# isarandi/smplfitter

Hardware: AMD Instinct MI355X
Metric: fits/sec (SMPL 6890-vert, 3 iters) (higher is better)
Workload: dtype f32; 1 GPU; SMPL-neutral (synthetic SMPL-shaped model) batch 4096/GPU, 6890 verts, num_iter=3, beta_reg=1, joints given; batch_per_gpu=4096, num_iter=3, parallelism=batch-sharded x1

## Files before the change

smplfitter_amd/csrc/kernels_wave.inc:

```
template <bool WEIGHTED>
__global__ __launch_bounds__(256) void k_center_sort_partsum(DevModel m, const float* __restrict__ tv,
                                                             const float* __restrict__ tj,
                                                             const float* __restrict__ vw,
                                                             Workspace ws) {
  extern __shared__ __attribute__((aligned(16))) float smem[];
  const int b = blockIdx.x, tid = threadIdx.x, lane = tid & 63, wave = tid >> 6;
  const int V = m.V, J = m.J, Vp = m.Vp;
  float(*red)[4] = reinterpret_cast<float(*)[4]>(smem + 4 * J * sf::kPsum);
  float* mu = smem + 4 * J * sf::kPsum + 16;
  const float* tvb = tv + (size_t)b * V * 3;
  float sx = 0.f, sy = 0.f, sz = 0.f;
  for (int v = tid; v < V; v += 256) {
    sx += tvb[v * 3];
    sy += tvb[v * 3 + 1];
    sz += tvb[v * 3 + 2];
  }
  if (tj) {
    for (int j = tid; j < J; j += 256) {
      sx += tj[((size_t)b * J + j) * 3];
      sy += tj[((size_t)b * J + j) * 3 + 1];
      sz += tj[((size_t)b * J + j) * 3 + 2];
    }
  }
  sx = wave_sum(sx);
// ... 333 lines not shown
      } else {
        acc[0][0] = __builtin_amdgcn_mfma_f32_32x32x2f32(a0, b0, acc[0][0], 0, 0, 0);
        acc[0][1] = __builtin_amdgcn_mfma_f32_32x32x2f32(a0, b1, acc[0][1], 0, 0, 0);
        acc[1][0] = __builtin_amdgcn_mfma_f32_32x32x2f32(a1, b0, acc[1][0], 0, 0, 0);
        acc[1][1] = __builtin_amdgcn_mfma_f32_32x32x2f32(a1, b1, acc[1][1], 0, 0, 0);
      }
    };
    __builtin_amdgcn_sched_group_barrier(0x100, 8, 0);
    mfma4(a0l.x, a1l.x, b0l.x, b1l.x);
    mfma4(a0l.y, a1l.y, b0l.y, b1l.y);
    mfma4(a0l.z, a1l.z, b0l.z, b1l.z);
    mfma4(a0l.w, a1l.w, b0l.w, b1l.w);
    mfma4(a0h.x, a1h.x, b0h.x, b1h.x);
    mfma4(a0h.y, a1h.y, b0h.y, b1h.y);
    mfma4(a0h.z, a1h.z, b0h.z, b1h.z);
    mfma4(a0h.w, a1h.w, b0h.w, b1h.w);
    if (it + 1 < nk) sstore(buf ^ 1);
    __syncthreads();
  }
#pragma unroll
  for (int mi = 0; mi < 2; ++mi)
#pragma unroll
    for (int ni = 0; ni < 2; ++ni)
#pragma unroll
      for (int r = 0; r < 16; ++r) {
        if (TRANSPOSED) {
          const int inst = m0 + wm + mi * 32 + l31;
          const int n = n0 + wn + ni * 32 + (r & 3) + 8 * (r >> 2) + 4 * lk;
          st_stream<2>(C + ((size_t)(inst >> 6) * N + n) * 64 + (inst & 63), acc[mi][ni][r]);
        } else {
          const int row = m0 + wm + mi * 32 + (r & 3) + 8 * (r >> 2) + 4 * lk;
          const int col = n0 + wn + ni * 32 + l31;
          st_stream<2>(C + (size_t)row * N + col, acc[mi][ni][r]);
        }
      }
}

constexpr int kNW = 4;

template <int NK2, bool TRANSPOSED>
__global__ __launch_bounds__(256, 2) void k_posedirs_gemm_as(const float* __restrict__ A,
                                                          const float* __restrict__ Bsw,
                                                          float* __restrict__ C, int N,
                                                          int tiles_per_chunk, int Mp) {
  constexpr int KP = 2 * NK2, RS = KP + 4;
  constexpr int TILE_F4 = 32 * KP / 4;
  constexpr int NQ = NK2 / 4;
  static_assert(NQ % 2 == 0, "the fragment reads alternate between two register quads");
  extern __shared__ __attribute__((aligned(16))) float smem[];
  const int tid = threadIdx.x, lane = tid & 63, wave = tid >> 6;
  const int l31 = lane & 31, lk = lane >> 5;
  const int m0 = (blockIdx.y * 4 + wave) * 32;
  const int ntiles = N / 32;
  const int t_begin = blockIdx.x * tiles_per_chunk;
  const int t_end = min(t_begin + tiles_per_chunk, ntiles);
  float a[NK2];
  {
    const float4* src = reinterpret_cast<const float4*>(A + (size_t)(m0 + l31) * KP + lk * NK2);
#pragma unroll
    for (int q = 0; q < NK2 / 4; ++q) {
      const float4 v = src[q];
      a[4 * q] = v.x; a[4 * q + 1] = v.y; a[4 * q + 2] = v.z; a[4 * q + 3] = v.w;
    }
  }
  static_assert(TILE_F4 <= 7 * 256, "tile too large for the staging registers");
  float4 s0, s1, s2, s3, s4, s5, s6;
#define SF_STAGE_ALL(OP) OP(0, s0) OP(1, s1) OP(2, s2) OP(3, s3) OP(4, s4) OP(5, s5) OP(6, s6)
  auto gload = [&](int tile) {
    const float4* src = reinterpret_cast<const float4*>(Bsw) + (size_t)tile * TILE_F4;
#define SF_LD(q, r)                                                       \
  if constexpr (256 * (q + 1) <= TILE_F4) r = src[tid + 256 * q];         \
  else if (tid + 256 * q < TILE_F4) r = src[tid + 256 * q];
    SF_STAGE_ALL(SF_LD)
#undef SF_LD
  };
  auto sstore = [&](int buf) {
    float* base = smem + (size_t)buf * 32 * RS;
#define SF_ST(q, r)                                                                        \
  if (256 * (q + 1) <= TILE_F4 || tid + 256 * q < TILE_F4) {                               \
    const int f = tid + 256 * q;                                                           \
    *reinterpret_cast<float4*>(base + (f / (KP / 4)) * RS + 4 * (f % (KP / 4))) = r;      \
  }
    SF_STAGE_ALL(SF_ST)
#undef SF_ST
  };
#undef SF_STAGE_ALL
  if (t_begin >= t_end) return;
  gload(t_begin);
  sstore(0);
  __syncthreads();
  for (int t = t_begin; t < t_end; ++t) {
    const int buf = (t - t_begin) & 1;
    if (t + 1 < t_end) gload(t + 1);
    f32x16 acc;
#pragma unroll
    for (int r = 0; r < 16; ++r) acc[r] = 0.f;
    const float4* brow = reinterpret_cast<const float4*>(smem + (size_t)buf * 32 * RS + l31 * RS + lk * NK2);
    auto mfma4 = [&](const float4& bq, int q) {
      if (TRANSPOSED) {
        acc = __builtin_amdgcn_mfma_f32_32x32x2f32(bq.x, a[4 * q], acc, 0, 0, 0);
        acc = __builtin_amdgcn_mfma_f32_32x32x2f32(bq.y, a[4 * q + 1], acc, 0, 0, 0);
        acc = __builtin_amdgcn_mfma_f32_32x32x2f32(bq.z, a[4 * q + 2], acc, 0, 0, 0);
        acc = __builtin_amdgcn_mfma_f32_32x32x2f32(bq.w, a[4 * q + 3], acc, 0, 0, 0);
      } else {
        acc = __builtin_amdgcn_mfma_f32_32x32x2f32(a[4 * q], bq.x, acc, 0, 0, 0);
        acc = __builtin_amdgcn_mfma_f32_32x32x2f32(a[4 * q + 1], bq.y, acc, 0, 0, 0);
        acc = __builtin_amdgcn_mfma_f32_32x32x2f32(a[4 * q + 2], bq.z, acc, 0, 0, 0);
        acc = __builtin_amdgcn_mfma_f32_32x32x2f32(a[4 * q + 3], bq.w, acc, 0, 0, 0);
      }
    };
    float4 bA = brow[0], bB;
    __builtin_amdgcn_sched_group_barrier(0x100, 1, 0);
#pragma unroll
    for (int q = 0; q < NQ; q += 2) {
      bB = brow[q + 1];
      __builtin_amdgcn_sched_group_barrier(0x100, 1, 0);
      mfma4(bA, q);
      __builtin_amdgcn_sched_group_barrier(0x008, 4, 0);
      if (q + 2 < NQ) bA = brow[q + 2];
      __builtin_amdgcn_sched_group_barrier(0x100, 1, 0);
      mfma4(bB, q + 1);
      __builtin_amdgcn_sched_group_barrier(0x008, 4, 0);
    }
    if (TRANSPOSED) {
      float* ccol = C + ((size_t)(m0 >> 6) * N + t * 32) * 64 + (m0 & 63) + l31;
#pragma unroll
      for (int r = 0; r < 16; ++r)
        st_stream<2>(ccol + (size_t)((r & 3) + 8 * (r >> 2) + 4 * lk) * 64, acc[r]);
    } else {
      float* crow = C + (size_t)m0 * N + t * 32 + l31;
#pragma unroll
      for (int r = 0; r < 16; ++r)
        st_stream<2>(crow + (size_t)((r & 3) + 8 * (r >> 2) + 4 * lk) * N, acc[r]);
    }
    if (t + 1 < t_end) sstore(buf ^ 1);
    __syncthreads();
  }
}

typedef __bf16 bf16x8 __attribute__((ext_vector_type(8)));
constexpr int kGemmKS = 13;
constexpr int kGemmPlaneBytes = 32 * 208 * 2;
constexpr int kGemmTileBytes = sf::kGemm3 ? 2 * kGemmPlaneBytes + 32 * 32 : 3 * kGemmPlaneBytes;
#ifndef SMPLFIT_GEMM_WAVES
#define SMPLFIT_GEMM_WAVES 8
#endif
constexpr int kGemmWaves = SMPLFIT_GEMM_WAVES;
#ifndef SMPLFIT_GEMM_RING
#define SMPLFIT_GEMM_RING 2
#endif
constexpr int kGemmRing = SMPLFIT_GEMM_RING;
static_assert(kGemmRing >= 2 && 16 * (kGemmRing - 1) + (kGemmRing - 2) * (kGemmTileBytes / 1024 / kGemmWaves + 1) <= 63,
              "s_waitcnt vmcnt is a 6-bit count");
template <int N>
__device__ __forceinline__ void wait_vmcnt() {
  asm volatile("s_waitcnt vmcnt(%0)" ::"n"(N) : "memory");
}
constexpr bool kGemm3 = sf::kGemm3;

__device__ __forceinline__ void lds_dma16(const char* src, uint32_t lane_off, char* lds) {
  const uint32_t l = (uint32_t)(uintptr_t)(__attribute__((address_space(3))) char*)lds;
  asm volatile("s_mov_b32 m0, %0\n\ts_nop 0\n\tglobal_load_lds_dwordx4 %1, %2" ::"s"(l), "v"(lane_off), "s"(src) : "memory", "m0");
}

template <bool TRANSPOSED>
__global__ __launch_bounds__(64 * kGemmWaves, 2) void k_posedirs_gemm_bf16x3(const float* __restrict__ A,
                                                                           const uint16_t* __restrict__ Bimg,
                                                                           float* __restrict__ C, int N,
                                                                           int tiles_per_chunk, int Mp) {
  constexpr int KS = kGemmKS, KP = 16 * KS, NW = kGemmWaves;
  constexpr int NDMA = kGemmTileBytes / 1024;
  extern __shared__ __attribute__((aligned(16))) char smem_b[];
  asm volatile("v_mov_b32 v255, 0" ::: "v255");
  const int tid = threadIdx.x, lane = tid & 63;
  const int wave = __builtin_amdgcn_readfirstlane(tid >> 6);
  const int l31 = lane & 31, kg = lane >> 5;
  const int m0 = (blockIdx.y * NW + wave) * 32;
  const bool active = m0 < Mp;
  const int ntiles = N / 32;
  const int t_begin = blockIdx.x * tiles_per_chunk;
  const int t_end = min(t_begin + tiles_per_chunk, ntiles);
  if (t_begin >= t_end) return;
  auto dma_tile = [&](int tile, int buf) {
    const char* src = reinterpret_cast<const char*>(Bimg) + (size_t)tile * kGemmTileBytes;
    char* dst = smem_b + buf * kGemmTileBytes;
#pragma unroll
    for (int i = 0; i < NDMA / NW; ++i) {
      const int c = wave + NW * i;
      lds_dma16(src + c * 1024, lane * 16, dst + c * 1024);
    }
    if (wave < NDMA % NW) {
      const int c = wave + NW * (NDMA / NW);
      lds_dma16(src + c * 1024, lane * 16, dst + c * 1024);
    }
  };
  constexpr int LEAD = kGemmRing - 1;
#pragma unroll
  for (int q = 0; q < LEAD; ++q) dma_tile(min(t_begin + q, t_end - 1), q);
  bf16x8 f1[KS], f2[KS], f3[KS];
  {
    const float* src = A + (size_t)((active ? m0 : 0) + l31) * KP + kg * 8;
#pragma unroll
    for (int s = 0; s < KS; ++s) {
      const float4 lo = *reinterpret_cast<const float4*>(src + 16 * s);
      const float4 hi = *reinterpret_cast<const float4*>(src + 16 * s + 4);
      const float x[8] = {lo.x, lo.y, lo.z, lo.w, hi.x, hi.y, hi.z, hi.w};
#pragma unroll
      for (int j = 0; j < 8; ++j) {
        const __bf16 h = (__bf16)x[j];
        const float r1 = x[j] - (float)h;
        const __bf16 m = (__bf16)r1;
        const __bf16 l = (__bf16)(r1 - (float)m);
        f1[s][j] = h;
        f2[s][j] = m;
        f3[s][j] = l;
      }
    }
  }
  const int frag_off = l31 * (KP * 2) + ((kg ^ ((l31 >> 3) & 1)) * 16);
  asm volatile("s_waitcnt vmcnt(0)" ::: "memory");
  __builtin_amdgcn_s_barrier();
  const bool extra = wave < NDMA % NW;
  int buf = 0, buf_req = LEAD;
  for (int t = t_begin; t < t_end; ++t) {
    const bool more = t + 1 < t_end;
    dma_tile(min(t + LEAD, t_end - 1), buf_req);
    if (active) {
      f32x16 acc;
#pragma unroll
      for (int r = 0; r < 16; ++r) acc[r] = 0.f;
      const char* base = smem_b + buf * kGemmTileBytes + frag_off;
      auto frag = [&](int plane, int s) {
        if constexpr (kGemm3) {
          if (plane == 2) return *reinterpret_cast<const bf16x8*>(smem_b + buf * kGemmTileBytes + 2 * kGemmPlaneBytes + l31 * 32 + kg * 16);
        }
        return *reinterpret_cast<const bf16x8*>(base + plane * kGemmPlaneBytes + s * 32);
      };
      auto mm = [&](const bf16x8& p, const bf16x8& f) {
        if (TRANSPOSED) acc = __builtin_amdgcn_mfma_f32_32x32x16_bf16(p, f, acc, 0, 0, 0);
        else acc = __builtin_amdgcn_mfma_f32_32x32x16_bf16(f, p, acc, 0, 0, 0);
      };
      bf16x8 p1 = frag(0, 0), p2 = frag(1, 0), p3 = p1;
      if constexpr (!kGemm3) p3 = frag(2, 0);
#pragma unroll
      for (int s = 0; s < KS; ++s) {
        bf16x8 n1, n2, n3;
        if (s + 1 < KS) {
          n1 = frag(0, s + 1);
          n2 = frag(1, s + 1);
          n3 = n1;
          if (!kGemm3 || s + 1 == KS - 1) n3 = frag(2, s + 1);
        }
        if constexpr (kGemm3) {
          if (s == KS - 1) mm(p3, f1[s]);
          mm(p2, f1[s]);
          mm(p1, f2[s]);
          mm(p1, f1[s]);
        } else {
          mm(p3, f1[s]);
          mm(p2, f2[s]);
          mm(p1, f3[s]);
          mm(p2, f1[s]);
          mm(p1, f2[s]);
          mm(p1, f1[s]);
        }
        if (s + 1 < KS) {
          p1 = n1;
          p2 = n2;
          p3 = n3;
        }
      }
      if (TRANSPOSED) {
        float* ccol = C + ((size_t)(m0 >> 6) * N + t * 32) * 64 + (m0 & 63) + l31;
#pragma unroll
        for (int r = 0; r < 16; ++r) st_stream<2>(ccol + (size_t)((r & 3) + 8 * (r >> 2) + 4 * kg) * 64, acc[r]);
      } else {
        float* crow = C + (size_t)m0 * N + t * 32 + l31;
#pragma unroll
        for (int r = 0; r < 16; ++r)
          st_stream<2>(crow + (size_t)((r & 3) + 8 * (r >> 2) + 4 * kg) * N, acc[r]);
      }
    }
    constexpr int N0 = (LEAD - 1) * (NDMA / NW), N1 = (LEAD - 1) * (NDMA / NW + 1), ST = 16 * LEAD;
    if (!more) wait_vmcnt<0>();
    else if (active) {
      if (extra) wait_vmcnt<ST + N1>();
      else wait_vmcnt<ST + N0>();
    } else {
      if (extra) wait_vmcnt<N1>();
      else wait_vmcnt<N0>();
    }
    __builtin_amdgcn_s_barrier();
    buf_req = buf;
    buf = buf + 1 == kGemmRing ? 0 : buf + 1;
  }
}

constexpr int kTgPlanesA = sf::kGemm3 ? 2 : 3;
constexpr int kTgStageA = kTgPlanesA * 256 * 64;
constexpr int kTgStageB = 3 * 128 * 64;
constexpr int kTgStage = kTgStageA + kTgStageB;

__global__ __launch_bounds__(256) void k_split_features(const float* __restrict__ A, uint16_t* __restrict__ img, int Mrows,
                                                        int Kp, int kc32) {
  const int mt = blockIdx.x, kc = blockIdx.y, r = threadIdx.x, row = mt * 256 + r;
  float x[32];
#pragma unroll
  for (int q = 0; q < 8; ++q) {
    const int k = kc * 32 + 4 * q;
    float4 v = make_float4(0.f, 0.f, 0.f, 0.f);
    if (row < Mrows && k + 3 < Kp) v = *reinterpret_cast<const float4*>(A + (size_t)row * Kp + k);
    else if (row < Mrows) {
      v.x = k < Kp ? A[(size_t)row * Kp + k] : 0.f;
      v.y = k + 1 < Kp ? A[(size_t)row * Kp + k + 1] : 0.f;
      v.z = k + 2 < Kp ? A[(size_t)row * Kp + k + 2] : 0.f;
    }
    x[4 * q] = v.x; x[4 * q + 1] = v.y; x[4 * q + 2] = v.z; x[4 * q + 3] = v.w;
  }
  uint16_t* base = img + ((size_t)mt * kc32 + kc) * (kTgStageA / 2);
#pragma unroll
  for (int sl = 0; sl < 4; ++sl) {
    bf16x8 h, m, l;
#pragma unroll
    for (int j = 0; j < 8; ++j) {
      const float v = x[sl * 8 + j];
      const __bf16 hh = (__bf16)v;
      const float r1 = v - (float)hh;
      const __bf16 mm = (__bf16)r1;
      h[j] = hh; m[j] = mm; l[j] = (__bf16)(r1 - (float)mm);
    }
    const int ps = sl ^ ((r >> 2) & 3);
    uint16_t* d = base + (size_t)r * 32 + ps * 8;
    *reinterpret_cast<bf16x8*>(d) = h;
    *reinterpret_cast<bf16x8*>(d + 256 * 32) = m;
    if constexpr (kTgPlanesA == 3) *reinterpret_cast<bf16x8*>(d + 2 * 256 * 32) = l;
  }
}

constexpr int kTg2B = 2 * 128 * 64;
constexpr int kTg2Bias = kTgStageA + 2 * kTg2B;
constexpr int kTg2Stage = kTg2Bias + 2 * 128 * 64;

__global__ __launch_bounds__(512, 1) void k_posedirs_gemm_bf16x3_tiled(const uint16_t* __restrict__ Aimg,
                                                                       const uint16_t* __restrict__ Bimg,
                                                                       float* __restrict__ C, int N, int Mp, int mt_count,
                                                                       int kc32, int bias_step) {
  static_assert(kGemm3 && kTgPlanesA == 2, "three-product form");
  extern __shared__ __attribute__((aligned(16))) char smem_b[];
  asm volatile("v_mov_b32 v255, 0" ::: "v255");
  const int tid = threadIdx.x, lane = tid & 63;
  const int wave = __builtin_amdgcn_readfirstlane(tid >> 6);
  const int l31 = lane & 31, kg = lane >> 5;
  const int xcd = blockIdx.x & 7, rr = blockIdx.x >> 3, mt_per = (mt_count + 7) / 8;
  const int mtile = (rr % mt_per) * 8 + xcd, ntile = rr / mt_per;
  if (mtile >= mt_count) return;
  const int wm = wave & 3, wn = wave >> 2;
  const char* asrc = reinterpret_cast<const char*>(Aimg) + (size_t)mtile * kc32 * kTgStageA;
  const char* bsrc = reinterpret_cast<const char*>(Bimg) + (size_t)(2 * ntile) * kc32 * kTgStageB;
  const size_t bhalf = (size_t)kc32 * kTgStageB;
  auto dma_pieces = [&](int kc, int buf, int i0, int i1) {
    char* dst = smem_b + buf * kTg2Stage;
#pragma unroll
    for (int i = i0; i < i1; ++i) {
      const int c = wave + 8 * i;
      const char* src = c < 32 ? asrc + (size_t)kc * kTgStageA + c * 1024
                               : bsrc + ((c - 32) >> 4) * bhalf + (size_t)kc * kTgStageB + ((c - 32) & 15) * 1024;
      lds_dma16(src, lane * 16, dst + c * 1024);
    }
    if (i1 == 8 && kc == bias_step / 2) {
#pragma unroll
      for (int i = 0; i < 2; ++i) {
        const int e = wave + 8 * i;
        lds_dma16(bsrc + (e >> 3) * bhalf + (size_t)kc * kTgStageB + kTg2B + (e & 7) * 1024, lane * 16, dst + kTg2Bias + e * 1024);
      }
    }
  };
  auto dma_stage = [&](int kc, int buf) { dma_pieces(kc, buf, 0, 8); };
  f32x16 acc[2][4];
#pragma unroll
  for (int i = 0; i < 2; ++i)
#pragma unroll
    for (int j = 0; j < 4; ++j)
#pragma unroll
      for (int r = 0; r < 16; ++r) acc[i][j][r] = 0.f;
  const int ra = wm * 64 + l31;
  const int aoff = ra * 64 + ((kg ^ ((ra >> 2) & 3)) * 16);
  const int boff = kTgStageA + wn * kTg2B + l31 * 64 + ((kg ^ ((l31 >> 2) & 3)) * 16);
  const int b3off = kTg2Bias + wn * (128 * 64) + l31 * 64 + ((kg ^ ((l31 >> 2) & 3)) * 16);
  struct Frags {
    bf16x8 a[2][2], b[4][2];
  };
  auto read_frags = [&](Frags& f, const char* base, int s2) {
#pragma unroll
    for (int p = 0; p < 2; ++p) {
#pragma unroll
      for (int i = 0; i < 2; ++i) f.a[i][p] = *reinterpret_cast<const bf16x8*>(base + (aoff ^ (s2 * 32)) + i * 2048 + p * (256 * 64));
#pragma unroll
      for (int j = 0; j < 4; ++j) f.b[j][p] = *reinterpret_cast<const bf16x8*>(base + (boff ^ (s2 * 32)) + j * 2048 + p * (128 * 64));
    }
  };
  auto mfma_step = [&](const Frags& f) {
#pragma unroll
    for (int i = 0; i < 2; ++i)
#pragma unroll
      for (int j = 0; j < 4; ++j) {
        f32x16 a = acc[i][j];
        a = __builtin_amdgcn_mfma_f32_32x32x16_bf16(f.b[j][1], f.a[i][0], a, 0, 0, 0);
        a = __builtin_amdgcn_mfma_f32_32x32x16_bf16(f.b[j][0], f.a[i][1], a, 0, 0, 0);
        a = __builtin_amdgcn_mfma_f32_32x32x16_bf16(f.b[j][0], f.a[i][0], a, 0, 0, 0);
        acc[i][j] = a;
      }
  };
  auto bias_term = [&](const Frags& f, const char* base, int s2) {
#pragma unroll
    for (int j = 0; j < 4; ++j) {
      const bf16x8 f3 = *reinterpret_cast<const bf16x8*>(base + (b3off ^ (s2 * 32)) + j * 2048);
#pragma unroll
      for (int i = 0; i < 2; ++i) acc[i][j] = __builtin_amdgcn_mfma_f32_32x32x16_bf16(f3, f.a[i][0], acc[i][j], 0, 0, 0);
    }
  };
  dma_stage(0, 0);
  asm volatile("s_waitcnt vmcnt(0)" ::: "memory");
  __builtin_amdgcn_s_barrier();
  if (kc32 > 1) dma_stage(1, 1);
  Frags fx, fy;
  read_frags(fx, smem_b, 0);
  auto first_half = [&](int kc, auto bias_c) {
    constexpr bool BIAS = decltype(bias_c)::value;
    const char* base = smem_b + (kc & 1) * kTg2Stage;
    read_frags(fy, base, 1);
    __builtin_amdgcn_sched_barrier(0);
    if constexpr (BIAS)
      if (2 * kc == bias_step) bias_term(fx, base, 0);
    mfma_step(fx);
    __builtin_amdgcn_sched_barrier(0);
    if constexpr (BIAS)
      if (2 * kc + 1 == bias_step) bias_term(fy, base, 1);
  };
  auto mfma_group = [&](const Frags& f, int q) {
#pragma unroll
    for (int i = 0; i < 2; ++i)
#pragma unroll
      for (int j = 0; j < 4; ++j)
        acc[i][j] = __builtin_amdgcn_mfma_f32_32x32x16_bf16(f.b[j][q == 0 ? 1 : 0], f.a[i][q == 1 ? 1 : 0], acc[i][j], 0, 0, 0);
  };
  auto stage = [&](int kc, auto bias_c) {
    first_half(kc, bias_c);
    asm volatile("s_waitcnt vmcnt(0) lgkmcnt(0)" ::: "memory");
// ... 688 lines not shown
```

smplfitter_amd/csrc/smplfit_hip.hip:

```cpp
#include <hip/hip_runtime.h>

#include <algorithm>
#include <atomic>

#include <cstdio>
#include <cstdlib>
#include <cstring>
#include <mutex>
#include <string>
#include <vector>
#include <type_traits>

#include "../../include/smplfit.h"
#include "sf_stages.h"
#include "sf_tables.h"

namespace {

thread_local std::string g_last_error;

int fail(int code, const std::string& msg) {
  g_last_error = msg;
  return code;
}

#define SF_HIP_TRY(expr)                                                                   \
  do {                                                                                     \
    hipError_t e_ = (expr);                                                                \
    if (e_ != hipSuccess)                                                                  \
      return fail(SMPLFIT_ERR_HIP, std::string(#expr) + ": " + hipGetErrorString(e_));     \
  } while (0)

struct DevModel {
  int V, J, S, P, Vp, Kp, KW, n_used, nseg;
  sf::JointTabs jt;
  const int32_t* perm;
  const int32_t* inv_slot;
  const int32_t* segments;
  const int32_t* part_seg_start;
  const float *vt, *dm, *sd, *wval, *pdSw, *j_template, *cpackA, *cpackB, *gblob;
  const uint16_t* pdB;
  const uint16_t* pdB2;
  int kc32;
  int gemm_exclusive;
  const int32_t* gtiles;
  int ngt;
  const uint32_t* widx;
  const int32_t *reg_start, *reg_slot;
  const float* reg_val;
  const float* reg_rowsum;
  int bm_tables;
  const float* brec;
  const float *pair_E, *pair_c2e, *diag_c2e;
  const int32_t *jn_start, *jn;
  int general;
  const float* sdg;
  const int32_t* segall;
  int nsegall;
  const int32_t *anc_start, *anc;
};

struct ShareView {
  const int32_t* piece_start;
  const int32_t* pieces;
  const int32_t *aux_start, *aux_rows;
  int ncells, nrows;
  int rec;
  int mult;
  int fine;
  int max_aux;
  const int32_t* aux_pad;
  int aux_pitch;
};

}

constexpr int kMaxChunks = 4;

constexpr int kRefMaxAdj = 16;
struct RefGroups { int8_t wave[kRefMaxAdj]; };

struct smplfit_handle {
  sf::HostTables t;
  DevModel d{};
  std::vector<ShareView> views;
  std::vector<void*> allocs;
  bool has_device = false;
  int refine_group_max = 0;
  RefGroups refine_groups{};
  int8_t rot_slots[64];
  int rot_nslots = 0, rot_toes_per_wave = 0;
  int gemm_vgprs = 0;
  hipStream_t side[kMaxChunks - 1] = {};
  hipEvent_t ev_fork = nullptr, ev_join[kMaxChunks - 1] = {};
  bool have_streams = false;
  mutable std::mutex mu;
};

struct smplfit_transfer {
  int v_in = 0, v_out = 0;
  std::vector<int32_t> indptr, indices;
  std::vector<float> values;
  int32_t *d_indptr = nullptr, *d_indices = nullptr;
  float* d_values = nullptr;
  bool negate_x = false;
};

struct smplfit_convert_plan {
  const smplfit_handle *in = nullptr, *out = nullptr;
  int nslab = 0;
  int32_t *d_oslot = nullptr, *d_start = nullptr, *d_islot = nullptr;
  float* d_w = nullptr;
  bool negate_x = false;
};

struct smplfit_flip_plan {
  smplfit_convert_plan conv;
  int32_t* d_perm = nullptr;
};

namespace {

__device__ __forceinline__ float wave_sum(float v) {
#pragma unroll
  for (int o = 32; o > 0; o >>= 1) v += __shfl_xor(v, o, 64);
  return v;
}

template <int CTRL, int ROW_MASK>
__device__ __forceinline__ float dpp_step(float v) {
  const int x = __builtin_amdgcn_update_dpp(0, __builtin_bit_cast(int, v), CTRL, ROW_MASK, 0xf, false);
  return v + __builtin_bit_cast(float, x);
}
__device__ __forceinline__ float wave_sum_last(float v) {
  v = dpp_step<0x111, 0xf>(v);
  v = dpp_step<0x112, 0xf>(v);
  v = dpp_step<0x114, 0xf>(v);
  v = dpp_step<0x118, 0xf>(v);
  v = dpp_step<0x142, 0xa>(v);
  v = dpp_step<0x143, 0xc>(v);
  return v;
}

struct DevCtx {
  int lane, n;
  __device__ __forceinline__ void sync() const { __syncthreads(); }
  __device__ __forceinline__ float sum_to_last(float v) const { return wave_sum_last(v); }
};

__device__ __forceinline__ float half_sum_last(float v) {
  v = dpp_step<0x111, 0xf>(v);
  v = dpp_step<0x112, 0xf>(v);
  v = dpp_step<0x114, 0xf>(v);
  v = dpp_step<0x118, 0xf>(v);
  v = dpp_step<0x142, 0xa>(v);
  return v;
}

struct DevCtxHalf {
  int lane, n;
  __device__ __forceinline__ void sync() const { __syncthreads(); }
  __device__ __forceinline__ float sum_to_last(float v) const { return half_sum_last(v); }
};
template <int N> struct StageCtx { using type = DevCtx; };
// ... 435 lines not shown
  do {                                                                         \
    if ((d).S == 10 && (d).KW == 4) { CALL(10, 4); }                           \
    else if ((d).S == 10 && (d).KW == 8) { CALL(10, 8); }                      \
    else if ((d).S == 16 && (d).KW == 4) { CALL(16, 4); }                      \
    else if ((d).S == 16 && (d).KW == 8) { CALL(16, 8); }                      \
    else if ((d).S == 11 && (d).KW == 4) { CALL(11, 4); }                      \
    else if ((d).S == 11 && (d).KW == 8) { CALL(11, 8); }                      \
    else if ((d).S == 17 && (d).KW == 4) { CALL(17, 4); }                      \
    else return fail(SMPLFIT_ERR_UNSUPPORTED,                                  \
                     "unsupported (shape unknowns, skinning width) combination"); \
  } while (0)

int launch_gen_accum_mfma(const DevModel& d, const Workspace& ws, int B, bool weighted, double* vextra, const float* tj,
                          const float* jw, hipStream_t st) {
  const size_t lds = gen2_lds(d.J, d.S, d.KW);
  if (lds > 160 * 1024) return fail(SMPLFIT_ERR_UNSUPPORTED, "general path: too many shape unknowns for the accumulate kernel's LDS tile");
  const bool stage = gen2_stage_joints(d.J, d.S, d.KW);
  const int nw = gen2_nw(d.S), nbw = gen2_nbw(d.S);
  const dim3 grid(B, gen2_groups(d.S));
  const int flush_every = vextra ? 1 : std::max(1, 2048 / gen2_sv(d.S));
#define SF_GEN2(W_, NW_, NBW_, ST_)                                                                                   \
  do {                                                                                                                \
    ensure_max_lds(reinterpret_cast<const void*>(&k_gen_accum_mfma<W_, NW_, NBW_, ST_>)); \
    hipLaunchKernelGGL((k_gen_accum_mfma<W_, NW_, NBW_, ST_>), grid, dim3(64 * NW_), lds, st, d, ws, B, vextra, flush_every, tj, jw); \
  } while (0)
#define SF_GEN2_W(NW_, NBW_, ST_)               \
  do {                                          \
    if (weighted) SF_GEN2(true, NW_, NBW_, ST_); \
    else SF_GEN2(false, NW_, NBW_, ST_);        \
  } while (0)
#define SF_GEN2_S(NW_, NBW_)              \
  do {                                    \
    if (stage) SF_GEN2_W(NW_, NBW_, true); \
    else SF_GEN2_W(NW_, NBW_, false);     \
  } while (0)
  if (nw == 4) SF_GEN2_S(4, 1);
  else if (nbw == 1) SF_GEN2_S(16, 1);
  else SF_GEN2_S(8, 7);
#undef SF_GEN2_S
#undef SF_GEN2_W
#undef SF_GEN2
  return 0;
}
bool gen_joint_rows(const DevModel& d) { return d.general && tune().gen_mfma; }
int launch_gen_accum(const DevModel& d, const Workspace& ws, int B, bool weighted, hipStream_t st, const float* jrows_tj,
                     const float* jrows_jw, bool extras) {
  if (tune().gen_mfma) return launch_gen_accum_mfma(d, ws, B, weighted, extras ? ws.gvex : nullptr, jrows_tj, jrows_jw, st);
  const size_t lds = gen_accum_lds(d.J, d.S, d.KW);
  if (lds > 160 * 1024) return fail(SMPLFIT_ERR_UNSUPPORTED, "general path: too many shape unknowns for the accumulate kernel's LDS tile");
  const bool stage = gen_accum_stage_joints(d.J, d.S, d.KW);
  const int tv = gen_tile_vertices(d.S), nt = gen_accum_threads(d.S);
#define SF_GEN(W_, TV_, NT_, ST_)                                                                              \
  do {                                                                                                         \
    ensure_max_lds(reinterpret_cast<const void*>(&k_gen_accum<W_, TV_, NT_, ST_>)); \
    hipLaunchKernelGGL((k_gen_accum<W_, TV_, NT_, ST_>), dim3(B), dim3(NT_), lds, st, d, ws, B);               \
  } while (0)
#define SF_GEN_W(TV_, NT_, ST_)              \
  do {                                       \
    if (weighted) SF_GEN(true, TV_, NT_, ST_); \
    else SF_GEN(false, TV_, NT_, ST_);       \
  } while (0)
#define SF_GEN_S(TV_, NT_)            \
  do {                                \
    if (stage) SF_GEN_W(TV_, NT_, true); \
    else SF_GEN_W(TV_, NT_, false);   \
  } while (0)
  if (nt == 64) SF_GEN_S(32, 64);
  else if (tv == 32) SF_GEN_S(32, 256);
  else SF_GEN_S(8, 256);
#undef SF_GEN_S
#undef SF_GEN_W
#undef SF_GEN
  return 0;
}
template <int MODE>
void launch_gen_lbs(const DevModel& d, const Workspace& ws, int B, bool weighted, int nb, const float* beta,
                    const float* trans, float* out, hipStream_t st, const float* kid = nullptr) {
  const size_t lds = gen_lbs_lds(d.J, d.S, B);
  const int ni = gen_lbs_ni(d.S, B);
#define SF_GLBS(M_, W_)                                                                                                   \
  do {                                                                                                                    \
    if (ni == 4) {                                                                                                        \
      ensure_max_lds(reinterpret_cast<const void*>(&k_gen_lbs<M_, W_, 4>));   \
      hipLaunchKernelGGL((k_gen_lbs<M_, W_, 4>), dim3((B + 3) / 4), dim3(256), lds, st, d, ws, B, nb, beta, trans, kid, out); \
    } else {                                                                                                              \
      hipLaunchKernelGGL((k_gen_lbs<M_, W_, 1>), dim3(B), dim3(256), lds, st, d, ws, B, nb, beta, trans, kid, out);       \
    }                                                                                                                     \
  } while (0)
  if (weighted && MODE != 2) SF_GLBS((MODE == 2 ? 0 : MODE), true);
  else SF_GLBS(MODE, false);
#undef SF_GLBS
}
int launch_accum_any(const DevModel& d, const Workspace& ws, int B, bool weighted, bool pair_form, hipStream_t st,
                     const float* jrows_tj = nullptr, const float* jrows_jw = nullptr, bool extras = false) {
  if (d.general) return launch_gen_accum(d, ws, B, weighted, st, jrows_tj, jrows_jw, extras);
#define SF_CALL_ACCUM(S_, KW_) launch_shape_accum<S_, KW_>(d, ws, B, weighted, pair_form, st)
  SF_DISPATCH_SKW(d, SF_CALL_ACCUM);
#undef SF_CALL_ACCUM
  return 0;
}
template <int MODE>
int launch_lbs_any(const DevModel& d, const Workspace& ws, int B, bool weighted, int nb, const float* beta,
                   const float* trans, float* out, hipStream_t st, const float* kid = nullptr) {
  if (d.general) {
    launch_gen_lbs<MODE>(d, ws, B, weighted, nb, beta, trans, out, st, kid);
    return 0;
  }
#define SF_CALL_LBS(S_, KW_) launch_lbs<S_, KW_, MODE, false>(d, ws, B, weighted, nb, beta, trans, out, 0.f, 0.f, st, kid)
  SF_DISPATCH_SKW(d, SF_CALL_LBS);
#undef SF_CALL_LBS
  return 0;
}

size_t chunked_workspace_bytes(const sf::HostTables& t, int batch, const sf::HostTables* tin = nullptr);

int check_common(const smplfit_handle* h, int batch, void* workspace, size_t workspace_bytes, bool bwd = false) {
  if (!h) return fail(SMPLFIT_ERR_BAD_ARG, bwd ? "smplfit_forward_backward_f32: null handle" : "null handle");
  if (!h->has_device) return fail(SMPLFIT_ERR_HIP, "handle was created host-only (no device)");
  if (batch <= 0) return fail(SMPLFIT_ERR_BAD_ARG, "batch must be positive");
  if (!workspace || ((uintptr_t)workspace & 255))
    return fail(SMPLFIT_ERR_WORKSPACE, "workspace must be a 256-byte aligned device pointer");
  if (bwd && workspace_bytes < smplfit_forward_backward_workspace_bytes(h, batch))
    return fail(SMPLFIT_ERR_WORKSPACE, "workspace too small (smplfit_forward_backward_workspace_bytes)");
  if (!bwd && workspace_bytes < chunked_workspace_bytes(h->t, batch))
    return fail(SMPLFIT_ERR_WORKSPACE, "workspace too small (see smplfit_workspace_bytes)");
  return 0;
}

int check_scale_share(const char* who, int scale_mode, const float* scale_corr, int share_beta,
                      smplfit_share_allreduce_fn share_allreduce) {
  if (scale_mode < 0 || scale_mode > 2)
    return fail(SMPLFIT_ERR_BAD_ARG, std::string(who) + ": scale_mode must be 0, 1 (scale_target) or 2 (scale_fit)");
  if (scale_mode && !scale_corr) return fail(SMPLFIT_ERR_BAD_ARG, std::string(who) + ": a scale option needs the scale_corr output");
  if (share_allreduce && !share_beta) return fail(SMPLFIT_ERR_BAD_ARG, std::string(who) + ": share_allreduce without share_beta");
  return 0;
}

int check_forward_inputs(const char* who, const DevModel& d, const float* pose, const float* glob, const float* rel,
                         const float* betas, int num_betas_given, const float* kid) {
  if ((pose != nullptr) + (glob != nullptr) + (rel != nullptr) > 1)
    return fail(SMPLFIT_ERR_BAD_ARG, "Only one rotation input may be provided");
  if (betas && num_betas_given > d.S - d.jt.n_kid - d.jt.n_pad)
    return fail(SMPLFIT_ERR_BAD_ARG, std::string(who) + ": more betas than the model holds; slice first");
  if (kid && !d.jt.n_kid) return fail(SMPLFIT_ERR_BAD_ARG, std::string(who) + ": kid_factor given to a handle without kid");
  return 0;
}

bool gemm_bf16x3() { return !tune().gemm_f32; }

int launch_gemm(const DevModel& d, const Workspace& ws, int B, hipStream_t st, bool transposed = false) {
  const int Mp = (int)align_up((size_t)B, 128), N = 3 * d.Vp;
  if (d.Kp == 208 && gemm_bf16x3() && d.gemm_exclusive) {
    const int ntiles = N / 32, ny = (Mp + 32 * kGemmWaves - 1) / (32 * kGemmWaves);
    const int nchunk = std::min(std::max(8, (2 * 256 / ny + 4) / 8 * 8), ntiles);
    const int per = (ntiles + nchunk - 1) / nchunk;
    const size_t lds = (size_t)kGemmRing * kGemmTileBytes;
    ensure_max_lds(reinterpret_cast<const void*>(&k_posedirs_gemm_bf16x3<true>));
    ensure_max_lds(reinterpret_cast<const void*>(&k_posedirs_gemm_bf16x3<false>));
    if (transposed)
      hipLaunchKernelGGL((k_posedirs_gemm_bf16x3<true>), dim3(nchunk, ny), dim3(64 * kGemmWaves), lds, st, ws.rp,
                         d.pdB, ws.vpT, N, per, Mp);
    else
      hipLaunchKernelGGL((k_posedirs_gemm_bf16x3<false>), dim3(nchunk, ny), dim3(64 * kGemmWaves), lds, st, ws.rp,
                         d.pdB, ws.vposed, N, per, Mp);
    return 0;
  }
  if (d.Kp != 208 && transposed && d.kc32 > 0 && gemm_bf16x3() && d.gemm_exclusive) {
    const int mt = (Mp + 255) / 256, nt256 = N / 256;
    uint16_t* aimg = reinterpret_cast<uint16_t*>(ws.vposed);
    hipLaunchKernelGGL(k_split_features, dim3(mt, d.kc32), dim3(256), 0, st, ws.rp, aimg, Mp, d.Kp, d.kc32);
    ensure_max_lds(reinterpret_cast<const void*>(&k_posedirs_gemm_bf16x3_tiled));
    hipLaunchKernelGGL(k_posedirs_gemm_bf16x3_tiled, dim3(8 * ((mt + 7) / 8) * nt256), dim3(512), (size_t)2 * kTg2Stage, st,
                       aimg, d.pdB2, ws.vpT, N, Mp, mt, d.kc32, sf::rp_pos(d.P, d.Kp) / 16);
    return 0;
  }
  if (d.Kp == 208) {
    constexpr int NK2 = 104;
    const int ntiles = N / 32;
    int nchunk = std::max(1, (3 * 256 + Mp / 128 - 1) / (Mp / 128));
    nchunk = std::min(nchunk, ntiles);
    const int per = (ntiles + nchunk - 1) / nchunk;
    nchunk = (ntiles + per - 1) / per;
    const size_t lds = (size_t)2 * 32 * (2 * NK2 + 4) * 4;
    if (transposed)
      hipLaunchKernelGGL((k_posedirs_gemm_as<NK2, true>), dim3(nchunk, Mp / 128), dim3(256), lds, st,
                         ws.rp, d.pdSw, ws.vpT, N, per, Mp);
    else
      hipLaunchKernelGGL((k_posedirs_gemm_as<NK2, false>), dim3(nchunk, Mp / 128), dim3(256), lds, st,
                         ws.rp, d.pdSw, ws.vposed, N, per, Mp);
    return 0;
  }
  if (transposed)
    hipLaunchKernelGGL(k_posedirs_gemm<true>, dim3((N / 128) * (Mp / 128)), dim3(256), 0, st, ws.rp, d.pdSw,
                       ws.vpT, Mp, N, d.Kp);
  else
    hipLaunchKernelGGL(k_posedirs_gemm<false>, dim3((N / 128) * (Mp / 128)), dim3(256), 0, st, ws.rp, d.pdSw,
                       ws.vposed, Mp, N, d.Kp);
  return 0;
}

size_t joint_lds(const DevModel& d, int kind = 0) {
  return (size_t)sf::joint_scratch_floats(d.J, d.general ? 0 : d.S, kind) * 4;
}
size_t solve_lds(const DevModel& d) {
  return d.general ? (size_t)(sf::kSolvePanel * d.S + sf::kSolvePanel) * 8 : (size_t)sf::solve_scratch_floats(d.S) * 4;
}

#ifndef SMPLFIT_STAGE_HALF
#define SMPLFIT_STAGE_HALF 7
#endif
inline bool stage_half(const DevModel& d, int bit, int B) {
  return (SMPLFIT_STAGE_HALF & bit) && d.J <= 32 && B >= tune().stage_half_b && !d.general;
}

void launch_forward_joint(const DevModel& d, const ForwardArgs& fa, const Workspace& ws, int B, hipStream_t st) {
  if (d.general) hipLaunchKernelGGL(k_forward_joint<true>, dim3(B), dim3(64), joint_lds(d), st, d, fa, ws);
  else hipLaunchKernelGGL(k_forward_joint<false>, dim3(B), dim3(64), joint_lds(d), st, d, fa, ws);
}
void launch_joint_stage(const DevModel& d, JointStageArgs ja, const Workspace& ws, int B, hipStream_t st) {
  ja.B = B;
  ja.b0 = 0;
  if (stage_half(d, 1, B)) {
    if (B / 2 > 0) hipLaunchKernelGGL(k_joint_stage<32>, dim3(B / 2), dim3(64), 2 * joint_lds(d), st, d, ja, ws);
    if (B & 1) {
      ja.b0 = B - 1;
      hipLaunchKernelGGL(k_joint_stage<64>, dim3(1), dim3(64), joint_lds(d), st, d, ja, ws);
    }
  } else {
    if (d.general) hipLaunchKernelGGL((k_joint_stage<64, true>), dim3(B), dim3(64), joint_lds(d), st, d, ja, ws);
    else hipLaunchKernelGGL(k_joint_stage<64>, dim3(B), dim3(64), joint_lds(d), st, d, ja, ws);
  }
}
void launch_refine(const DevModel& d, RefineArgs ra, const Workspace& ws, int B, hipStream_t st) {
  ra.B = B;
  ra.b0 = 0;
  if (stage_half(d, 4, B)) {
    if (B / 2 > 0) hipLaunchKernelGGL(k_refine_epilogue<32>, dim3(B / 2), dim3(64), 2 * joint_lds(d, 1), st, d, ra, ws);
    if (B & 1) {
      ra.b0 = B - 1;
      hipLaunchKernelGGL(k_refine_epilogue<64>, dim3(1), dim3(64), joint_lds(d, 1), st, d, ra, ws);
    }
  } else {
    hipLaunchKernelGGL(k_refine_epilogue<64>, dim3(B), dim3(64), joint_lds(d, 1), st, d, ra, ws);
  }
}
void launch_shape_solve(const DevModel& d, const Workspace& ws, int B, hipStream_t st, float beta_reg, float beta_reg2,
                        float kid_reg, int pair_form, int use_ref, int mode = 0, int first = 0, int count = -1,
                        int cen_b0 = 0) {
  if (count < 0) count = B;
  if (d.general) {
    ensure_max_lds(reinterpret_cast<const void*>(&k_shape_solve<64, true>));
    hipLaunchKernelGGL((k_shape_solve<64, true>), dim3(count), dim3(d.S > 128 ? 1024 : d.S > 64 ? 256 : 64), solve_lds(d), st, d,
                       ws, B, beta_reg, beta_reg2, kid_reg, pair_form, use_ref, mode, first, cen_b0);
  } else if (stage_half(d, 2, B)) {
    if (B / 2 > 0)
      hipLaunchKernelGGL(k_shape_solve<32>, dim3(B / 2), dim3(64), 2 * solve_lds(d), st, d, ws, B, beta_reg,
                         beta_reg2, kid_reg, pair_form, use_ref, mode, 0, 0);
    if (B & 1)
      hipLaunchKernelGGL(k_shape_solve<64>, dim3(1), dim3(64), solve_lds(d), st, d, ws, B, beta_reg, beta_reg2,
                         kid_reg, pair_form, use_ref, mode, B - 1, 0);
  } else {
    hipLaunchKernelGGL(k_shape_solve<64>, dim3(B), dim3(64), solve_lds(d), st, d, ws, B, beta_reg, beta_reg2,
                       kid_reg, pair_form, use_ref, mode, 0, 0);
  }
}

constexpr int kSolveIB = 16;
struct SolveBmPlan {
  bool ok = false;
  SolveBmArgs a{};
  ShareView sv{};
  size_t lds = 0;
};
SolveBmPlan solve_bm_plan(const smplfit_handle* h, int B) {
  SolveBmPlan p;
  const DevModel& d = h->d;
  if (d.general || !(d.S == 10 || d.S == 11) || !d.bm_tables) return p;
  const int idx = share_index(sf::kShareResidual, B);
  if (idx >= sf::kShareFine || (size_t)idx >= h->views.size()) return p;
  const sf::ShareTable& t = h->t.shares[idx];
  const int maxn = h->views[idx].aux_pitch;
  const size_t Mp = align_up((size_t)B, 128);
  const size_t res_rows = (size_t)t.ncells * ((d.S + 3 + 3) / 4 * 4) + (size_t)t.nrows * 3 * sf::kGroupJoints;
  const size_t res_bytes = res_rows * Mp * 4;
  const size_t gram_bytes = (size_t)pair_gram_workgroups(d.J, d.jt.np) * sf::ne_ng(d.S) * Mp * 4;
  const size_t jdt_bytes = Mp * align_up((size_t)d.J * sf::jd_stride(d.S), 64) * 4;
  int lg = 0;
  while ((8 << lg) < t.ncells) ++lg;
  if (maxn > kSolveT3 || (8 << lg) != t.ncells || res_bytes >= (1u << 31) || gram_bytes >= (1u << 31) || jdt_bytes >= (1u << 31) ||
      !h->views[idx].aux_pad)
    return p;
  p.sv = share_view(h, sf::kShareResidual, B);
  const bool stage_px = solve_bm_lds_bytes(d.S, kSolveIB, d.J, t.ncells, maxn, true) <= 156 * 1024;
  p.lds = solve_bm_lds_bytes(d.S, kSolveIB, d.J, t.ncells, maxn, stage_px);
  if (p.lds > 156 * 1024) return p;
  p.a.stage_px = stage_px ? 1 : 0;
  p.a.maxn = maxn;
  p.a.lg_ngrp = lg;
  p.a.res_bytes = (uint32_t)res_bytes;
  p.a.gram_bytes = (uint32_t)gram_bytes;
  p.a.jdt_bytes = (uint32_t)jdt_bytes;
  p.ok = true;
  return p;
}
template <int S>
void launch_solve_bm_s(const smplfit_handle* h, const Workspace& ws, int B, hipStream_t st, SolveBmPlan p) {
  const DevModel& d = h->d;
// ... 1825 lines not shown
```

Before: 2.801 million fits/s.

## Overlap posedirs GEMM output stores with next tile's MFMAs via software pipelining

Restructures the bf16x3 posedirs GEMM loop into a two-accumulator pipeline. The previous tile's 16 streaming stores are interleaved, through sched_group_barrier, with the current tile's MFMA chain, and the first LDS fragments are loaded before issuing the next DMA. The goal is to hide global store latency and the exposed epilogue behind tensor-core work. The vmcnt waits are adjusted for the stores now in flight. The launch also halves the chunk count, so each block handles more tiles and amortises the prologue, at the cost of fewer blocks in flight and more register pressure from the second accumulator.

After: 2.800 million fits/s. About the same (-0.0%).

```diff
diff --git a/smplfitter_amd/csrc/kernels_wave.inc b/smplfitter_amd/csrc/kernels_wave.inc
--- a/smplfitter_amd/csrc/kernels_wave.inc
+++ b/smplfitter_amd/csrc/kernels_wave.inc
@@ -509,6 +509,14 @@
 constexpr int kGemmRing = SMPLFIT_GEMM_RING;
 static_assert(kGemmRing >= 2 && 16 * (kGemmRing - 1) + (kGemmRing - 2) * (kGemmTileBytes / 1024 / kGemmWaves + 1) <= 63,
               "s_waitcnt vmcnt is a 6-bit count");
+template <int... I, class F>
+__device__ __forceinline__ void static_for_seq(std::integer_sequence<int, I...>, F&& f) {
+  (f(std::integral_constant<int, I>{}), ...);
+}
+template <int N, class F>
+__device__ __forceinline__ void static_for(F&& f) {
+  static_for_seq(std::make_integer_sequence<int, N>{}, f);
+}
 template <int N>
 __device__ __forceinline__ void wait_vmcnt() {
   asm volatile("s_waitcnt vmcnt(%0)" ::"n"(N) : "memory");
@@ -579,34 +587,49 @@
   __builtin_amdgcn_s_barrier();
   const bool extra = wave < NDMA % NW;
   int buf = 0, buf_req = LEAD;
-  for (int t = t_begin; t < t_end; ++t) {
+  float* const cbase = TRANSPOSED ? C + (size_t)(m0 >> 6) * N * 64 + (m0 & 63) + l31 + 4 * kg * 64
+                                  : C + ((size_t)m0 + 4 * kg) * N + l31;
+  auto store1 = [&](const f32x16& a, int t, int r) {
+    const int row = (r & 3) + 8 * (r >> 2);
+    if (TRANSPOSED) st_stream<2>(cbase + ((size_t)t * 32 + row) * 64, a[r]);
+    else st_stream<2>(cbase + (size_t)row * N + t * 32, a[r]);
+  };
+  auto step = [&](f32x16& acc, const f32x16& prev, auto has_prev, int t) {
+    constexpr bool HAS_PREV = decltype(has_prev)::value;
     const bool more = t + 1 < t_end;
-    dma_tile(min(t + LEAD, t_end - 1), buf_req);
+    const char* base = smem_b + buf * kGemmTileBytes + frag_off;
+    const char* base3 = smem_b + buf * kGemmTileBytes + 2 * kGemmPlaneBytes + l31 * 32 + kg * 16;
+    auto frag = [&](int plane, int s) {
+      if constexpr (kGemm3) {
+        if (plane == 2) return *reinterpret_cast<const bf16x8*>(base3);
+      }
+      return *reinterpret_cast<const bf16x8*>(base + plane * kGemmPlaneBytes + s * 32);
+    };
+    bf16x8 p1, p2, p3;
     if (active) {
-      f32x16 acc;
+      p1 = frag(0, 0);
+      p2 = frag(1, 0);
+      p3 = p1;
+      if constexpr (!kGemm3) p3 = frag(2, 0);
+    }
+    if (more) dma_tile(min(t + LEAD, t_end - 1), buf_req);
+    if (active) {
 #pragma unroll
       for (int r = 0; r < 16; ++r) acc[r] = 0.f;
-      const char* base = smem_b + buf * kGemmTileBytes + frag_off;
-      auto frag = [&](int plane, int s) {
-        if constexpr (kGemm3) {
-          if (plane == 2) return *reinterpret_cast<const bf16x8*>(smem_b + buf * kGemmTileBytes + 2 * kGemmPlaneBytes + l31 * 32 + kg * 16);
-        }
-        return *reinterpret_cast<const bf16x8*>(base + plane * kGemmPlaneBytes + s * 32);
-      };
       auto mm = [&](const bf16x8& p, const bf16x8& f) {
         if (TRANSPOSED) acc = __builtin_amdgcn_mfma_f32_32x32x16_bf16(p, f, acc, 0, 0, 0);
         else acc = __builtin_amdgcn_mfma_f32_32x32x16_bf16(f, p, acc, 0, 0, 0);
       };
-      bf16x8 p1 = frag(0, 0), p2 = frag(1, 0), p3 = p1;
-      if constexpr (!kGemm3) p3 = frag(2, 0);
-#pragma unroll
-      for (int s = 0; s < KS; ++s) {
+      static_for<KS>([&](auto sc) {
+        constexpr int s = decltype(sc)::value;
         bf16x8 n1, n2, n3;
-        if (s + 1 < KS) {
+        constexpr int NREAD = s + 1 < KS ? (!kGemm3 || s + 1 == KS - 1 ? 3 : 2) : 0;
+        if constexpr (NREAD >= 2) {
           n1 = frag(0, s + 1);
           n2 = frag(1, s + 1);
           n3 = n1;
-          if (!kGemm3 || s + 1 == KS - 1) n3 = frag(2, s + 1);
+          if constexpr (NREAD == 3) n3 = frag(2, s + 1);
+          __builtin_amdgcn_sched_group_barrier(0x100, NREAD, 0);
         }
         if constexpr (kGemm3) {
           if (s == KS - 1) mm(p3, f1[s]);
@@ -621,28 +644,31 @@
           mm(p1, f2[s]);
           mm(p1, f1[s]);
         }
-        if (s + 1 < KS) {
+        constexpr int NMM = kGemm3 ? (s == KS - 1 ? 4 : 3) : 6;
+        constexpr int r0 = 16 * s / KS, r1 = 16 * (s + 1) / KS;
+        __builtin_amdgcn_sched_group_barrier(0x008, 1, 0);
+        if constexpr (HAS_PREV && r1 > r0) {
+#pragma unroll
+          for (int r = r0; r < r1; ++r) store1(prev, t - 1, r);
+          __builtin_amdgcn_sched_group_barrier(0x040, r1 - r0, 0);
+        }
+        __builtin_amdgcn_sched_group_barrier(0x008, NMM - 1, 0);
+        if constexpr (s + 1 < KS) {
           p1 = n1;
           p2 = n2;
           p3 = n3;
         }
-      }
-      if (TRANSPOSED) {
-        float* ccol = C + ((size_t)(m0 >> 6) * N + t * 32) * 64 + (m0 & 63) + l31;
-#pragma unroll
-        for (int r = 0; r < 16; ++r) st_stream<2>(ccol + (size_t)((r & 3) + 8 * (r >> 2) + 4 * kg) * 64, acc[r]);
-      } else {
-        float* crow = C + (size_t)m0 * N + t * 32 + l31;
-#pragma unroll
-        for (int r = 0; r < 16; ++r)
-          st_stream<2>(crow + (size_t)((r & 3) + 8 * (r >> 2) + 4 * kg) * N, acc[r]);
-      }
-    }
-    constexpr int N0 = (LEAD - 1) * (NDMA / NW), N1 = (LEAD - 1) * (NDMA / NW + 1), ST = 16 * LEAD;
-    if (!more) wait_vmcnt<0>();
-    else if (active) {
+      });
+    }
+    if (!more) return;
+    constexpr int N0 = (LEAD - 1) * (NDMA / NW), N1 = (LEAD - 1) * (NDMA / NW + 1);
+    constexpr int ST = HAS_PREV ? 16 * LEAD : 0, ST1 = HAS_PREV ? 16 : 0;
+    if (active && t - t_begin >= LEAD) {
       if (extra) wait_vmcnt<ST + N1>();
       else wait_vmcnt<ST + N0>();
+    } else if (active) {
+      if (extra) wait_vmcnt<ST1 + N1>();
+      else wait_vmcnt<ST1 + N0>();
     } else {
       if (extra) wait_vmcnt<N1>();
       else wait_vmcnt<N0>();
@@ -650,7 +676,27 @@
     __builtin_amdgcn_s_barrier();
     buf_req = buf;
     buf = buf + 1 == kGemmRing ? 0 : buf + 1;
-  }
+  };
+  constexpr std::false_type kFirst{};
+  constexpr std::true_type kNext{};
+  f32x16 acc0, acc1;
+  step(acc0, acc0, kFirst, t_begin);
+  int t = t_begin + 1;
+  for (; t + 1 < t_end; t += 2) {
+    step(acc1, acc0, kNext, t);
+    step(acc0, acc1, kNext, t + 1);
+  }
+  if (t < t_end) {
+    step(acc1, acc0, kNext, t);
+    if (active) {
+#pragma unroll
+      for (int r = 0; r < 16; ++r) store1(acc1, t, r);
+    }
+  } else if (active) {
+#pragma unroll
+    for (int r = 0; r < 16; ++r) store1(acc0, t - 1, r);
+  }
+  wait_vmcnt<0>();
 }
 
 constexpr int kTgPlanesA = sf::kGemm3 ? 2 : 3;
diff --git a/smplfitter_amd/csrc/smplfit_hip.hip b/smplfitter_amd/csrc/smplfit_hip.hip
--- a/smplfitter_amd/csrc/smplfit_hip.hip
+++ b/smplfitter_amd/csrc/smplfit_hip.hip
@@ -10,6 +10,7 @@
 #include <string>
 #include <vector>
 #include <type_traits>
+#include <utility>
 
 #include "../../include/smplfit.h"
 #include "sf_stages.h"
@@ -751,7 +752,7 @@
   const int Mp = (int)align_up((size_t)B, 128), N = 3 * d.Vp;
   if (d.Kp == 208 && gemm_bf16x3() && d.gemm_exclusive) {
     const int ntiles = N / 32, ny = (Mp + 32 * kGemmWaves - 1) / (32 * kGemmWaves);
-    const int nchunk = std::min(std::max(8, (2 * 256 / ny + 4) / 8 * 8), ntiles);
+    const int nchunk = std::min(std::max(8, (256 / ny + 4) / 8 * 8), ntiles);
     const int per = (ntiles + nchunk - 1) / nchunk;
     const size_t lds = (size_t)kGemmRing * kGemmTileBytes;
     ensure_max_lds(reinterpret_cast<const void*>(&k_posedirs_gemm_bf16x3<true>));
```
